# rmcar17/SpectralClusterSupertree

Hardware: AMD Instinct MI355X
Metric: top-level PCG build + Fiedler solve wall-time (s) at N taxa, 1/2/4/8 MI355X (lower is better)
Workload: dtype f64 (loop operator: fp32 image of W; fp64 renewal + confirmation)

## Files before the change

spectralclustersupertree_amd/csrc/scs_eig.hip:

```cpp

#include <algorithm>
#include <chrono>
#include <cmath>

#include "scs_internal.h"
#include "scs_policy.h"
#include "scs_symm.h"
#include "scs_matfree.h"
#include "scs_symm_tri.h"

#include <sched.h>
#include "scs_panel.h"

constexpr int MAXB = 16;
constexpr int MAXS = 64;
constexpr int SLD = MAXS + 1;

typedef double v4d __attribute__((ext_vector_type(4)));

__global__ void k_scale_rows(const double *__restrict__ x, int ldx, int c0, int b, int n,
                             const double *__restrict__ dinv, double *__restrict__ zt,
                             int64_t ldz) {
    const int idx = blockIdx.x * blockDim.x + threadIdx.x;
    if (idx >= n * b) return;
// ... 111 lines not shown
                                                          int nparts, int nout,
                                                          double *__restrict__ out) {
    const int lane = threadIdx.x & 63;
    const int e = blockIdx.x * 4 + (threadIdx.x >> 6);
    if (e >= nout) return;
    double s = 0.0;
    for (int p = lane; p < nparts; p += 64) s += partial[(int64_t)p * nout + e];
#pragma unroll
    for (int o = 32; o > 0; o >>= 1) s += __shfl_xor(s, o, 64);
    if (lane == 0) out[e] = s;
}

__global__ __launch_bounds__(256) void k_update(double *y, int ldy, int kc, double alpha_y,
                                                 const double *a, int lda, int ka,
                                                 const double *__restrict__ c, int ldc,
                                                 double sign, int n) {
    __shared__ double sc[3 * MAXB][MAXB];
    for (int e = threadIdx.x; e < ka * kc; e += 256) {
        const int i = e / kc, j = e - i * kc;
        sc[i][j] = c[i * ldc + j];
    }
    __syncthreads();
    const int r = blockIdx.x * 16 + (threadIdx.x >> 4);
    const int j = threadIdx.x & 15;
    double acc = 0.0, yold = 0.0;
    const bool live = r < n && j < kc;
    if (live) {
        const double *ar = a + (int64_t)r * lda;
        for (int i = 0; i < ka; ++i) acc += ar[i] * sc[i][j];
        if (alpha_y != 0.0) yold = y[(int64_t)r * ldy + j];
    }
    __syncthreads();
// ... 69 lines not shown
    x ^= x >> 30;
    x *= 0xBF58476D1CE4E5B9ull;
    x ^= x >> 27;
    x *= 0x94D049BB133111EBull;
    x ^= x >> 31;
    return (double)(x >> 11) * (2.0 / 9007199254740992.0) - 1.0;
}

__global__ void k_init_block(double *__restrict__ q, int b, int n, const double *__restrict__ x0) {
    const int idx = blockIdx.x * blockDim.x + threadIdx.x;
    if (idx >= n * b) return;
    const int i = idx / b, k = idx - i * b;
    double v = hash_uniform((unsigned long long)i, (unsigned long long)k + 1);
    if (k == 0 && x0) v = x0[i];
    q[(int64_t)i * (3 * b) + k] = v;
}

__global__ void k_fill_int(int *p, int n, int v) {
    const int i = blockIdx.x * blockDim.x + threadIdx.x;
    if (i < n) p[i] = v;
}

__global__ void k_trivial(const double *__restrict__ deg, double inv_norm, int n,
                          double *__restrict__ u) {
    const int i = blockIdx.x * blockDim.x + threadIdx.x;
    if (i < n) u[i] = sqrt(deg[i]) * inv_norm;
}

__global__ void k_extract_maps(const double *__restrict__ q, int ldq, int n,
                               const double *__restrict__ dinv, double inv_norm, int constrained,
                               double *__restrict__ out) {
    const int i = blockIdx.x * blockDim.x + threadIdx.x;
    if (i >= n) return;
    const double di = dinv[i];
    if (constrained) {
// ... 857 lines not shown
        const int i = e / b, k = e - i * b;
        double v = 0.0;
        for (int a = 0; a < b; ++a) v += dd[i][a] * gg[a][k];
        d[e] = v;
    }
}

__global__ __launch_bounds__(256) void k_small_rr(const double *__restrict__ tm, int nparts,
                                                   int nq, int b, const int *__restrict__ mask,
                                                   double *__restrict__ c, double *__restrict__ d,
                                                   double *__restrict__ theta,
                                                   int *__restrict__ mask_p, double drop_tol) {
    small_rr_body(tm, nparts, nq, b, mask, c, d, theta, mask_p, drop_tol);
}

struct orth_lds {
    jacobi_lds s;
    double cxp[16][8], gm[9][8], mm[8][8], tt[8][8], dsc[8];
    double tmp[8][3 * MAXB * 3 * MAXB / 4];
    __device__ void eig(int b) { jacobi_eig(s, b); }
};
template <int B>
struct orth_small_lds {
    jacobi_small_lds<B> s;
    double cxp[2 * B][B], gm[B + 1][B], mm[B][B], tt[B][B], dsc[B];
    double tmp[8][3 * B * B + B];
    double coef[PANEL_COEF_ROWS<B> * B];
    panel_red_t red;
    __device__ void eig(int) { jacobi_eig_waves<B>(s); }
};
// ... 86 lines not shown
template <int B>
__global__ __launch_bounds__(256) void k_panel_rr_solve(double *q, double *aq,
                                                         const double *__restrict__ u,
                                                         const double *__restrict__ tm, int nparts_in,
                                                         int solve, double *theta_g,
                                                         const int *__restrict__ maskp_in,
                                                         const int *__restrict__ mask_r,
                                                         int *maskp_out, double drop_tol, int n,
                                                         double *__restrict__ partial,
                                                         const double *__restrict__ dinv = nullptr,
                                                         double *__restrict__ zt = nullptr, int64_t ldz = 0,
                                                         int exact_from = -1) {
    __shared__ double c_s[3 * B * B], d_s[3 * B * B], th_s[B + 4];
    __shared__ int live_s[3 * B], mp_s[B];
    const int tid = threadIdx.x;
    if (solve) {
        if (tid < 3 * B) live_s[tid] = tid < B ? 1 : (tid < 2 * B ? maskp_in[tid - B] : mask_r[tid - 2 * B]);
        __syncthreads();
        small_rr_body(tm, nparts_in, 3 * B, B, live_s, c_s, d_s, th_s, mp_s, drop_tol, exact_from);
    } else {
        for (int e = tid; e < 3 * B * B; e += 256) {
            c_s[e] = (e / B == e % B) ? 1.0 : 0.0;
            d_s[e] = 0.0;
        }
        if (tid <= B) th_s[tid] = theta_g[tid];
        if (tid < B) mp_s[tid] = 0;
    }
    __syncthreads();
    if (blockIdx.x == 0) {
        if (solve && tid <= B) theta_g[tid] = th_s[tid];
        if (tid < B) maskp_out[tid] = mp_s[tid];
    }
    panel_rr_body<B>(q, aq, u, c_s, d_s, th_s, n, partial, dinv, zt, ldz);
}

template <int B, bool GRAM, bool WRITE_Z>
__global__ __launch_bounds__(256) void k_panel_tf_solve(double *q, const double *__restrict__ u,
                                                         const double *__restrict__ part_in,
                                                         int nparts_in, double drop_tol, int *mask_r,
                                                         const double *__restrict__ theta_g,
                                                         double *report, double seq, int n,
                                                         double *__restrict__ partial,
                                                         const double *__restrict__ dinv,
                                                         double *__restrict__ zt, int64_t ldz) {
    __shared__ double coef_s[PANEL_COEF_ROWS<B> * B];
    const bool lead = blockIdx.x == 0;
    small_orth_body(part_in, nparts_in, B, drop_tol, coef_s, lead ? mask_r : nullptr, theta_g,
                    lead ? report : nullptr, -1.0);
    __syncthreads();
    panel_tf_body<B, GRAM, WRITE_Z>(q, u, coef_s, n, partial, dinv, zt, ldz);
    if (lead && report) {
        __threadfence_system();
        __syncthreads();
        if (threadIdx.x == 0) ((volatile double *)report)[40] = seq;
    }
}

template <int B, int FINISH>
__global__ __launch_bounds__(256) void k_panel_gram_tf_solve(double *q, double *aq, const double *__restrict__ u,
                                                              const double *__restrict__ part_in, int nparts_in,
                                                              int *mask_r, const double *__restrict__ theta_g, int n,
                                                              const double *__restrict__ ypart, int nseg,
                                                              const double *__restrict__ dinv,
                                                              double *__restrict__ partial, int64_t chunk = 0,
                                                              const int32_t *__restrict__ splits = nullptr,
                                                              const double *__restrict__ coef1 = nullptr) {
    constexpr int NC = PANEL_COEF_ROWS<B> * B;
    __shared__ double coef_s[NC], coefa_s[NC];
    const bool lead = blockIdx.x == 0;
    small_orth_body(part_in, nparts_in, B, 0.0, coef_s, lead ? mask_r : nullptr, theta_g, nullptr, -1.0);
    __syncthreads();
    for (int e = threadIdx.x; e < NC; e += 256) {
        const int k = e / B, c = e - k * B;
        double v = coef_s[e];
        if (coef1) {
            if (k >= 2 * B && k < 3 * B) v = 0.0;
            for (int i = 0; i < B; ++i) v += coef1[k * B + i] * coef_s[(2 * B + i) * B + c];
        }
        coefa_s[e] = v;
    }
    __syncthreads();
    panel_gram_tf_body<B, FINISH>(q, aq, u, coef_s, coefa_s, n, ypart, nseg, dinv, partial, chunk, splits);
}

template <int B, int CT, int RPW, int D, typename WT = double>
__global__ __launch_bounds__(256, 2) void k_symm_tri_tf(const WT *__restrict__ w, int64_t ld, int n,
                                                        const double *__restrict__ zt, int64_t ldz,
                                                        const int2 *__restrict__ tiles,
                                                        double *__restrict__ pdir, double *__restrict__ ptr_,
                                                        int n_tf, double *q, const double *__restrict__ u,
                                                        const double *__restrict__ part_in, int nparts_in,
                                                        double drop_tol, int *mask_r,
                                                        const double *__restrict__ theta_g, double *report,
                                                        double seq, double *__restrict__ partial,
                                                        double *__restrict__ coef_out) {
    union lds_t {
        symm_tri_lds<B, CT, WT> symm;
        orth_small_lds<B> tf;
    };
    __shared__ lds_t lds;
    const int bid = blockIdx.x;
    if (bid >= n_tf) {
        symm_tri_body<B, CT, RPW, D, WT>(w, ld, n, zt, ldz, tiles[bid - n_tf], pdir, ptr_, 0, lds.symm);
        return;
    }
    const bool lead = bid == 0;
    small_orth_core(lds.tf, part_in, nparts_in, B, drop_tol, lds.tf.coef, lead ? mask_r : nullptr, theta_g,
                    lead ? report : nullptr, -1.0);
    __syncthreads();
    if (lead)
        for (int e = threadIdx.x; e < PANEL_COEF_ROWS<B> * B; e += 256) coef_out[e] = lds.tf.coef[e];
    panel_tf_body<B, true, false>(q, u, lds.tf.coef, n, partial, nullptr, nullptr, 0, bid, n_tf, &lds.tf.red);
    if (lead && report) {
        __threadfence_system();
        __syncthreads();
        if (threadIdx.x == 0) ((volatile double *)report)[40] = seq;
    }
}

__global__ void k_unit_coeffs(double *__restrict__ c, double *__restrict__ d, int b) {
    const int e = blockIdx.x * blockDim.x + threadIdx.x;
    if (e >= 3 * b * b) return;
    c[e] = (e / b == e % b) ? 1.0 : 0.0;
    d[e] = 0.0;
}

__global__ void k_dense_s(const double *__restrict__ w, int64_t ld, int n,
// ... 521 lines not shown
        k_gram_mfma<TA, TB><<<nparts, 64, 0, s>>>(a, lda, ka, bm, ldb, kb, n, part.d());
            GM(1, 1) GM(1, 2) GM(1, 3) GM(2, 1) GM(2, 2) GM(2, 3) GM(3, 1) GM(3, 2) GM(3, 3)
#undef GM
        } else {
            nparts = std::min(gram_blocks, std::max(1, (n + GRAM_CH - 1) / GRAM_CH));
            k_gram<<<nparts, 256, 0, s>>>(a, lda, ka, bm, ldb, kb, n, part.d());
        }
        k_reduce_partials<<<(nout + 3) / 4, 256, 0, s>>>(part.d(), nparts, nout, out);
        SCS_HIP_CHECK(hipGetLastError());
        return SCS_OK;
    }

    int update(double *y, int ldy, int kc, double alpha, const double *a, int lda, int ka,
               const double *c, int ldc, double sign) {
        k_update<<<(n + 15) / 16, 256, 0, s>>>(y, ldy, kc, alpha, a, lda, ka, c, ldc, sign, n);
        SCS_HIP_CHECK(hipGetLastError());
        return SCS_OK;
    }

    static int panel_cap() {
        static const int cap = PANEL_BLOCKS_MAX;
        return cap;
    }
    int panel_blocks16() const { return std::max(1, std::min(panel_cap(), ((n + 15) / 16 + 3) / 4)); }
    int panel_blocks4() const { return std::max(1, std::min(panel_cap(), ((n + 3) / 4 + 3) / 4)); }

    template <int B>
    int fused_front(const double *uvec, const double *c, const double *d, const double *theta,
                    double *coef, int *mask_r, double drop_tol, double *report, double seq) {
        const int nb = panel_blocks16();
// ... 356 lines not shown
        for (int pass = 0; pass < 2; ++pass) {
            SCS_TRY(sv.gram(Y, q3, b, Y, q3, b, G, sv.use_mfma));
            k_small_svqb<<<1, 256, 0, s>>>(G, b, pass == 0 ? drop_tol : 0.0, T, mask_out);
            SCS_TRY(sv.update(Y, q3, b, 0.0, Y, q3, b, T, b, 1.0));
            if (AY) SCS_TRY(sv.update(AY, q3, b, 0.0, AY, q3, b, T, b, 1.0));
        }
        return SCS_OK;
    };

    k_init_block<<<(n * b + 255) / 256, 256, 0, s>>>(Q, b, n, x_init ? x0d.d() : nullptr);
    SCS_TRY(project_u(X, 2));
    SCS_TRY(svqb(X, nullptr, MASK));
    SCS_TRY(sv.apply(Q, 0, AQ, 0));
    SCS_TRY(sv.gram(X, q3, b, AX, q3, b, G, sv.use_mfma));
    {
        k_fill_int<<<1, 64, 0, s>>>(MASK, 48, 1);
        k_small_rr<<<1, 256, 0, s>>>(G, 0, b, b, MASK, T, D, TH, MASK + b, drop_tol);
        SCS_TRY(sv.update(X, q3, b, 0.0, X, q3, b, T, b, 1.0));
        SCS_TRY(sv.update(AX, q3, b, 0.0, AX, q3, b, T, b, 1.0));
        k_fill_int<<<1, 64, 0, s>>>(MASK + b, b, 0);
    }

    const int res_blocks = (n + 255) / 256;
    dbuf res_part;
    SCS_TRY(res_part.alloc((size_t)res_blocks * b * 8));
    std::vector<double> h_rn(b), h_th(b + 1);
    int iter = 0;
    bool converged = false;
    double final_res[2] = {0.0, 0.0};

    const bool fused = (b == 4 || b == 8) &&
                       !(scs_dbg("SCS_LEGACY_LOOP") && atoi(scs_dbg("SCS_LEGACY_LOOP")));
    if (fused) {
        if (!ctx->h_report) {
            SCS_HIP_CHECK(hipHostMalloc((void **)&ctx->h_report, 64 * sizeof(double),
// ... 87 lines not shown
        }
        const int action = policy.step(worst);
        const bool stop = action == scs_loop_policy::STOP;
        if (action == scs_loop_policy::RENEW) {
            sv.use32 = false;
            SCS_TRY(sv.apply(Q, 0, AQ, 0));
            SCS_TRY(sv.apply(Q, b, AQ, b));
            sv.use32 = policy.image_in_use();
            ++st->lowp_renewals;
        }
        if (stop) {
            sv.use32 = false;
            if (policy.begin_confirmation()) {
                SCS_TRY(sv.apply(Q, 0, AQ, 0));
                SCS_TRY(sv.gram(X, q3, b, AX, q3, b, G, sv.use_mfma));
                k_fill_int<<<1, 64, 0, s>>>(MASK, 48, 1);
                k_small_rr<<<1, 256, 0, s>>>(G, 0, b, b, MASK, T, D, TH, MASK + b, drop_tol);
                SCS_TRY(sv.update(X, q3, b, 0.0, X, q3, b, T, b, 1.0));
                SCS_TRY(sv.update(AX, q3, b, 0.0, AX, q3, b, T, b, 1.0));
                k_fill_int<<<1, 64, 0, s>>>(MASK + b, b, 0);
                k_residual<<<res_blocks, 256, 0, s>>>(Q, AQ, b, TH, n, res_part.d());
                k_reduce_partials<<<(b + 3) / 4, 256, 0, s>>>(res_part.d(), res_blocks, b, RN);
                SCS_HIP_CHECK(hipMemcpyAsync(h_rn.data(), RN, (size_t)b * 8, hipMemcpyDeviceToHost, s));
                SCS_HIP_CHECK(hipMemcpyAsync(h_th.data(), TH, (size_t)(b + 1) * 8,
                                             hipMemcpyDeviceToHost, s));
                SCS_HIP_CHECK(hipStreamSynchronize(s));
                double w2 = 0.0;
                for (int j = 0; j < want; ++j) w2 = std::max(w2, std::sqrt(h_rn[j]));
                for (int j = 0; j < want; ++j) final_res[constrained ? 1 : j] = std::sqrt(h_rn[j]);
                bool conv = false;
                if (policy.confirm(w2, &conv)) {
                    converged = conv;
                    break;
                }
                if (fused) k_unit_coeffs<<<(3 * b * b + 255) / 256, 256, 0, s>>>(T, D, b);
// ... 1287 lines not shown
```

spectralclustersupertree_amd/csrc/scs_panel.h:

```cpp
#pragma once
#include <hip/hip_runtime.h>

#include <cstdint>

typedef double panel_v4d __attribute__((ext_vector_type(4)));

constexpr int PANEL_BLOCKS_MAX = 128;

template <int B>
struct panel_out {
    static constexpr int XP = 2 * B * B;
    static constexpr int RU = (B + 1) * B;
    static constexpr int TOTAL = XP + RU;
};

template <int B>
constexpr int PANEL_COEF_ROWS = 3 * B + 4;

typedef double panel_red_t[4][2][4][64];

template <int B>
__device__ __forceinline__ void panel_store_partials(panel_v4d g1, panel_v4d g2,
                                                     double *__restrict__ partial, int bid = -1,
                                                     panel_red_t *red_ext = nullptr) {
// ... 11 lines not shown
    if (wave == 0) {
        double *out = partial + (int64_t)bid * panel_out<B>::TOTAL;
#pragma unroll
        for (int r = 0; r < 4; ++r) {
            const int i = kk + 4 * r;
            const double s1 = ((red[0][0][r][lane] + red[1][0][r][lane]) + red[2][0][r][lane]) +
                              red[3][0][r][lane];
            const double s2 = ((red[0][1][r][lane] + red[1][1][r][lane]) + red[2][1][r][lane]) +
                              red[3][1][r][lane];
            if (i < 2 * B && cc < B) out[i * B + cc] = s1;
            if (i <= B && cc < B) out[panel_out<B>::XP + i * B + cc] = s2;
        }
    }
}

template <int B>
__device__ __forceinline__ void panel_rr_body(double *q, double *aq, const double *__restrict__ u,
                                              const double *c, const double *d, const double *theta,
                                              int n, double *__restrict__ partial,
                                              const double *__restrict__ dinv = nullptr,
                                              double *__restrict__ zt = nullptr, int64_t ldz = 0) {
    static_assert(B == 4 || B == 8, "fused panel kernels take block widths 4 and 8");
    constexpr int LD = 3 * B;
    const int lane = threadIdx.x & 63, wave = threadIdx.x >> 6;
    const int kk = lane >> 4, cc = lane & 15;
    const int n_groups = (n + 15) / 16;
    panel_v4d g1 = {0.0, 0.0, 0.0, 0.0}, g2 = {0.0, 0.0, 0.0, 0.0};
    const double th = cc < B ? theta[cc] : 0.0;
    double coef[LD / 4];
#pragma unroll
    for (int k = 0; k < LD / 4; ++k) {
        const int row = 4 * k + kk;
        coef[k] = cc < B ? c[row * B + cc] : (cc < 2 * B ? d[row * B + cc - B] : 0.0);
    }
    for (int grp = blockIdx.x * 4 + wave; grp < n_groups; grp += gridDim.x * 4) {
        const int base = grp * 16;
        const int ra = base + cc;
        panel_v4d dq = {0.0, 0.0, 0.0, 0.0}, da = {0.0, 0.0, 0.0, 0.0};
        double aq_op[LD / 4], q_op[LD / 4];
#pragma unroll
        for (int k = 0; k < LD / 4; ++k) {
            q_op[k] = ra < n ? q[(int64_t)ra * LD + 4 * k + kk] : 0.0;
            aq_op[k] = ra < n ? aq[(int64_t)ra * LD + 4 * k + kk] : 0.0;
        }
        double u_in[4];
#pragma unroll
        for (int r = 0; r < 4; ++r) {
            const int row = base + kk + 4 * r;
            u_in[r] = (cc == B && u && row < n) ? u[row] : 0.0;
        }
#pragma unroll
        for (int k = 0; k < LD / 4; ++k) {
            dq = __builtin_amdgcn_mfma_f64_16x16x4f64(q_op[k], coef[k], dq, 0, 0, 0);
            da = __builtin_amdgcn_mfma_f64_16x16x4f64(aq_op[k], coef[k], da, 0, 0, 0);
        }
#pragma unroll
        for (int r = 0; r < 4; ++r) {
            const int row = base + kk + 4 * r;
            const bool live = row < n;
            const double res = cc < B ? da[r] - dq[r] * th : 0.0;
            double ru = res;
            if (cc == B) ru = u_in[r];
            if (live && cc < 2 * B) {
                q[(int64_t)row * LD + cc] = dq[r];
                aq[(int64_t)row * LD + cc] = da[r];
            }
            if (live && cc < B) {
                q[(int64_t)row * LD + 2 * B + cc] = res;
                if (zt) zt[(int64_t)cc * ldz + row] = dinv[row] * res;
            }
            g1 = __builtin_amdgcn_mfma_f64_16x16x4f64(dq[r], res, g1, 0, 0, 0);
            g2 = __builtin_amdgcn_mfma_f64_16x16x4f64(ru, res, g2, 0, 0, 0);
        }
    }
    panel_store_partials<B>(g1, g2, partial);
}

template <int B>
__global__ __launch_bounds__(256) void k_panel_rr(double *q, double *aq,
                                                   const double *__restrict__ u,
                                                   const double *__restrict__ c,
                                                   const double *__restrict__ d,
                                                   const double *__restrict__ theta, int n,
                                                   double *__restrict__ partial) {
    panel_rr_body<B>(q, aq, u, c, d, theta, n, partial);
}

template <int B, bool GRAM, bool WRITE_Z>
__device__ __forceinline__ void panel_tf_body(double *q, const double *__restrict__ u,
                                              const double *coefm, int n,
                                              double *__restrict__ partial,
                                              const double *__restrict__ dinv,
                                              double *__restrict__ zt, int64_t ldz, int bid = -1,
                                              int nblk = -1, panel_red_t *red_ext = nullptr) {
    static_assert(B == 4 || B == 8, "fused panel kernels take block widths 4 and 8");
    constexpr int LD = 3 * B;
    constexpr int KC = PANEL_COEF_ROWS<B> / 4;
    if (bid < 0) {
        bid = blockIdx.x;
        nblk = gridDim.x;
    }
    const int lane = threadIdx.x & 63, wave = threadIdx.x >> 6;
    const int kk = lane >> 4, cc = lane & 15;
    const int n_groups = (n + 15) / 16;
    panel_v4d g1 = {0.0, 0.0, 0.0, 0.0}, g2 = {0.0, 0.0, 0.0, 0.0};
    double coef[KC];
#pragma unroll
    for (int k = 0; k < KC; ++k) coef[k] = cc < B ? coefm[(4 * k + kk) * B + cc] : 0.0;
    for (int grp = bid * 4 + wave; grp < n_groups; grp += nblk * 4) {
        const int base = grp * 16;
        const int ra = base + cc;
        double a_op[KC];
#pragma unroll
        for (int k = 0; k < KC - 1; ++k) a_op[k] = ra < n ? q[(int64_t)ra * LD + 4 * k + kk] : 0.0;
        a_op[KC - 1] = (kk == 0 && u && ra < n) ? u[ra] : 0.0;
        double xp_in[4], u_in[4];
        if (GRAM) {
#pragma unroll
            for (int r = 0; r < 4; ++r) {
                const int row = base + kk + 4 * r;
                xp_in[r] = (row < n && cc < 2 * B) ? q[(int64_t)row * LD + cc] : 0.0;
                u_in[r] = (cc == B && u && row < n) ? u[row] : 0.0;
            }
        }
        panel_v4d dr = {0.0, 0.0, 0.0, 0.0};
#pragma unroll
        for (int k = 0; k < KC; ++k)
            dr = __builtin_amdgcn_mfma_f64_16x16x4f64(a_op[k], coef[k], dr, 0, 0, 0);
#pragma unroll
        for (int r = 0; r < 4; ++r) {
            const int row = base + kk + 4 * r;
            const bool live = row < n;
            const double res = dr[r];
            if (live && cc < B) {
                q[(int64_t)row * LD + 2 * B + cc] = res;
                if (WRITE_Z) zt[(int64_t)cc * ldz + row] = dinv[row] * res;
            }
            if (GRAM) {
                const double xp = xp_in[r];
                double ru = res;
                if (cc == B) ru = u_in[r];
                g1 = __builtin_amdgcn_mfma_f64_16x16x4f64(xp, res, g1, 0, 0, 0);
                g2 = __builtin_amdgcn_mfma_f64_16x16x4f64(ru, res, g2, 0, 0, 0);
            }
        }
    }
    if (GRAM) panel_store_partials<B>(g1, g2, partial, bid, red_ext);
}

template <int B, bool GRAM, bool WRITE_Z>
__global__ __launch_bounds__(256) void k_panel_tf(double *q, const double *__restrict__ u,
                                                   const double *__restrict__ coefm, int n,
                                                   double *__restrict__ partial,
                                                   const double *__restrict__ dinv,
                                                   double *__restrict__ zt, int64_t ldz) {
    panel_tf_body<B, GRAM, WRITE_Z>(q, u, coefm, n, partial, dinv, zt, ldz);
}

template <int B, int FINISH>
__global__ __launch_bounds__(256) void k_gram_qaq(const double *__restrict__ q, double *aq, int n,
                                                   const double *__restrict__ ypart, int nseg,
                                                   const double *__restrict__ dinv,
// ... 79 lines not shown
#pragma unroll
        for (int i = 0; i < NT; ++i)
#pragma unroll
            for (int j = 0; j < NT; ++j)
#pragma unroll
                for (int r = 0; r < 4; ++r) {
                    const int t = i * NT + j;
                    const double s = ((red[0][t][r][lane] + red[1][t][r][lane]) + red[2][t][r][lane]) +
                                     red[3][t][r][lane];
                    const int orow = i * 16 + kk + 4 * r, ocol = j * 16 + cc;
                    if (orow < LD && ocol < LD) out[orow * LD + ocol] = s;
                }
    }
}

template <int B, int FINISH>
__device__ __forceinline__ void panel_gram_tf_body(double *q, double *aq, const double *__restrict__ u,
                                                   const double *coefm, const double *coefam, int n,
                                                   const double *__restrict__ ypart, int nseg,
                                                   const double *__restrict__ dinv,
                                                   double *__restrict__ partial, int64_t chunk,
                                                   const int32_t *__restrict__ splits) {
    static_assert(B == 4 || B == 8, "fused panel kernels take block widths 4 and 8");
    constexpr int LD = 3 * B;
    constexpr int KC = PANEL_COEF_ROWS<B> / 4;
    constexpr int NT = (LD + 15) / 16;
    constexpr int RT = (2 * B) / 16;
    constexpr int RC0 = 2 * B - 16 * RT;
    __shared__ double red[4][NT * NT][4][64];
    const int lane = threadIdx.x & 63, wave = threadIdx.x >> 6;
    const int kk = lane >> 4, cc = lane & 15;
    const int n_groups = (n + 15) / 16;
    panel_v4d acc[NT][NT];
#pragma unroll
    for (int i = 0; i < NT; ++i)
#pragma unroll
        for (int j = 0; j < NT; ++j) acc[i][j] = (panel_v4d){0.0, 0.0, 0.0, 0.0};
    double coef[KC], coefa[KC];
#pragma unroll
    for (int k = 0; k < KC; ++k) {
        const bool rc = cc >= RC0 && cc < RC0 + B;
        coef[k] = rc ? coefm[(4 * k + kk) * B + (cc - RC0)] : 0.0;
        coefa[k] = rc ? coefam[(4 * k + kk) * B + (cc - RC0)] : 0.0;
    }
    for (int grp = blockIdx.x * 4 + wave; grp < n_groups; grp += gridDim.x * 4) {
        const int base = grp * 16;
        const int ra = base + cc;
        double q_op[KC], a_op[KC];
#pragma unroll
        for (int k = 0; k < KC - 1; ++k) {
            const int col = 4 * k + kk;
            q_op[k] = ra < n ? q[(int64_t)ra * LD + col] : 0.0;
            double v = 0.0;
            if (ra < n) {
                if (col < 2 * B || FINISH == 0) {
                    v = aq[(int64_t)ra * LD + col];
                } else if (FINISH == 1) {
                    const int64_t idx = (int64_t)ra * B + (col - 2 * B);
                    double part[4];
#pragma unroll
                    for (int g = 0; g < 4; ++g) part[g] = g < nseg ? ypart[(int64_t)g * n * B + idx] : 0.0;
                    v = dinv[ra] * (((part[0] + part[1]) + part[2]) + part[3]);
                } else if (FINISH == 2) {
                    int r = 0;
                    while (r + 1 < nseg && ra >= splits[r + 1]) ++r;
                    v = ypart[(int64_t)r * chunk + (int64_t)(ra - splits[r]) * B + (col - 2 * B)];
                } else {
                    const int64_t idx = (int64_t)ra * B + (col - 2 * B);
                    double sum = 0.0;
                    for (int g = 0; g < nseg; ++g) sum += ypart[(int64_t)g * n * B + idx];
                    v = dinv[ra] * sum;
                }
            }
            a_op[k] = v;
        }
        {
            const double uu = (kk == 0 && u && ra < n) ? u[ra] : 0.0;
            q_op[KC - 1] = uu;
            a_op[KC - 1] = uu;
        }
        double xq[NT][4], xa[NT][4];
#pragma unroll
        for (int t = 0; t < NT; ++t)
#pragma unroll
            for (int r = 0; r < 4; ++r) {
                const int row = base + kk + 4 * r, col = t * 16 + cc;
                const bool live = row < n && col < 2 * B;
                xq[t][r] = live ? q[(int64_t)row * LD + col] : 0.0;
                xa[t][r] = live ? aq[(int64_t)row * LD + col] : 0.0;
            }
        panel_v4d dr = {0.0, 0.0, 0.0, 0.0}, da = {0.0, 0.0, 0.0, 0.0};
#pragma unroll
        for (int k = 0; k < KC; ++k) {
            dr = __builtin_amdgcn_mfma_f64_16x16x4f64(q_op[k], coef[k], dr, 0, 0, 0);
            da = __builtin_amdgcn_mfma_f64_16x16x4f64(a_op[k], coefa[k], da, 0, 0, 0);
        }
#pragma unroll
        for (int r = 0; r < 4; ++r) {
            const int row = base + kk + 4 * r;
            const bool rcol = cc >= RC0 && cc < RC0 + B;
            if (row < n && rcol) {
                q[(int64_t)row * LD + 2 * B + (cc - RC0)] = dr[r];
                aq[(int64_t)row * LD + 2 * B + (cc - RC0)] = da[r];
            }
            double fq[NT], fa[NT];
#pragma unroll
            for (int t = 0; t < NT; ++t) {
                fq[t] = xq[t][r];
                fa[t] = xa[t][r];
            }
            if (rcol) {
                fq[RT] = row < n ? dr[r] : 0.0;
                fa[RT] = row < n ? da[r] : 0.0;
            }
#pragma unroll
            for (int i = 0; i < NT; ++i)
#pragma unroll
                for (int j = 0; j < NT; ++j)
                    acc[i][j] = __builtin_amdgcn_mfma_f64_16x16x4f64(fq[i], fa[j], acc[i][j], 0, 0, 0);
        }
    }
#pragma unroll
    for (int i = 0; i < NT; ++i)
#pragma unroll
        for (int j = 0; j < NT; ++j)
#pragma unroll
            for (int r = 0; r < 4; ++r) red[wave][i * NT + j][r][lane] = acc[i][j][r];
    __syncthreads();
    if (wave == 0) {
        double *out = partial + (int64_t)blockIdx.x * LD * LD;
#pragma unroll
        for (int i = 0; i < NT; ++i)
#pragma unroll
            for (int j = 0; j < NT; ++j)
#pragma unroll
// ... 10 lines not shown
```

Measured before the change: 0.01418.

## Prefetch panel operands before the small Rayleigh-Ritz solve and fuse start-up kernels

The fused panel kernels now issue global loads for their first two row groups into registers before running the single-block small eigen/orthogonalisation solve, so memory latency overlaps that serial phase. The load and compute halves of the panel bodies are split into separate helpers to allow this. Separately, the start-up and confirmation Rayleigh-Ritz steps merge the mask fills and small solve into one kernel, and the two basis rotations into a single two-slice launch, cutting launch count. The cost is extra register pressure from holding the prefetched operands, which may reduce occupancy.

```diff
diff --git a/spectralclustersupertree_amd/csrc/scs_eig.hip b/spectralclustersupertree_amd/csrc/scs_eig.hip
--- a/spectralclustersupertree_amd/csrc/scs_eig.hip
+++ b/spectralclustersupertree_amd/csrc/scs_eig.hip
@@ -149,8 +149,13 @@
 __global__ __launch_bounds__(256) void k_update(double *y, int ldy, int kc, double alpha_y,
                                                  const double *a, int lda, int ka,
                                                  const double *__restrict__ c, int ldc,
-                                                 double sign, int n) {
+                                                 double sign, int n, double *y2 = nullptr,
+                                                 const double *a2 = nullptr) {
     __shared__ double sc[3 * MAXB][MAXB];
+    if (blockIdx.y) {
+        y = y2;
+        a = a2;
+    }
     for (int e = threadIdx.x; e < ka * kc; e += 256) {
         const int i = e / kc, j = e - i * kc;
         sc[i][j] = c[i * ldc + j];
@@ -250,11 +255,6 @@
     double v = hash_uniform((unsigned long long)i, (unsigned long long)k + 1);
     if (k == 0 && x0) v = x0[i];
     q[(int64_t)i * (3 * b) + k] = v;
-}
-
-__global__ void k_fill_int(int *p, int n, int v) {
-    const int i = blockIdx.x * blockDim.x + threadIdx.x;
-    if (i < n) p[i] = v;
 }
 
 __global__ void k_trivial(const double *__restrict__ deg, double inv_norm, int n,
@@ -1142,6 +1142,16 @@
     small_rr_body(tm, nparts, nq, b, mask, c, d, theta, mask_p, drop_tol);
 }
 
+__global__ __launch_bounds__(256) void k_small_rr_start(const double *__restrict__ tm, int b, int *mask,
+                                                         double *__restrict__ c, double *__restrict__ d,
+                                                         double *__restrict__ theta, double drop_tol) {
+    if (threadIdx.x < 48) mask[threadIdx.x] = 1;
+    __syncthreads();
+    small_rr_body(tm, 0, b, b, mask, c, d, theta, mask + b, drop_tol);
+    __syncthreads();
+    if ((int)threadIdx.x < b) mask[b + threadIdx.x] = 0;
+}
+
 struct orth_lds {
     jacobi_lds s;
     double cxp[16][8], gm[9][8], mm[8][8], tt[8][8], dsc[8];
@@ -1258,6 +1268,8 @@
     __shared__ double c_s[3 * B * B], d_s[3 * B * B], th_s[B + 4];
     __shared__ int live_s[3 * B], mp_s[B];
     const int tid = threadIdx.x;
+    panel_rr_ops<B> pre[PANEL_PRE];
+    panel_rr_prefetch<B>(pre, q, aq, u, dinv, zt != nullptr, n);
     if (solve) {
         if (tid < 3 * B) live_s[tid] = tid < B ? 1 : (tid < 2 * B ? maskp_in[tid - B] : mask_r[tid - 2 * B]);
         __syncthreads();
@@ -1275,7 +1287,7 @@
         if (solve && tid <= B) theta_g[tid] = th_s[tid];
         if (tid < B) maskp_out[tid] = mp_s[tid];
     }
-    panel_rr_body<B>(q, aq, u, c_s, d_s, th_s, n, partial, dinv, zt, ldz);
+    panel_rr_run<B>(pre, q, aq, u, c_s, d_s, th_s, n, partial, dinv, zt, ldz);
 }
 
 template <int B, bool GRAM, bool WRITE_Z>
@@ -1289,10 +1301,12 @@
                                                          double *__restrict__ zt, int64_t ldz) {
     __shared__ double coef_s[PANEL_COEF_ROWS<B> * B];
     const bool lead = blockIdx.x == 0;
+    panel_tf_ops<B> pre[PANEL_PRE];
+    panel_tf_prefetch<B, GRAM, WRITE_Z>(pre, q, u, dinv, n);
     small_orth_body(part_in, nparts_in, B, drop_tol, coef_s, lead ? mask_r : nullptr, theta_g,
                     lead ? report : nullptr, -1.0);
     __syncthreads();
-    panel_tf_body<B, GRAM, WRITE_Z>(q, u, coef_s, n, partial, dinv, zt, ldz);
+    panel_tf_run<B, GRAM, WRITE_Z>(pre, q, u, coef_s, n, partial, dinv, zt, ldz);
     if (lead && report) {
         __threadfence_system();
         __syncthreads();
@@ -1312,6 +1326,8 @@
     constexpr int NC = PANEL_COEF_ROWS<B> * B;
     __shared__ double coef_s[NC], coefa_s[NC];
     const bool lead = blockIdx.x == 0;
+    panel_gram_tf_ops<B> pre[PANEL_PRE];
+    panel_gram_tf_prefetch<B, FINISH>(pre, q, aq, u, n, ypart, nseg, dinv, chunk, splits);
     small_orth_body(part_in, nparts_in, B, 0.0, coef_s, lead ? mask_r : nullptr, theta_g, nullptr, -1.0);
     __syncthreads();
     for (int e = threadIdx.x; e < NC; e += 256) {
@@ -1324,7 +1340,7 @@
         coefa_s[e] = v;
     }
     __syncthreads();
-    panel_gram_tf_body<B, FINISH>(q, aq, u, coef_s, coefa_s, n, ypart, nseg, dinv, partial, chunk, splits);
+    panel_gram_tf_body<B, FINISH>(pre, q, aq, u, coef_s, coefa_s, n, ypart, nseg, dinv, partial, chunk, splits);
 }
 
 template <int B, int CT, int RPW, int D, typename WT = double>
@@ -1349,12 +1365,16 @@
         return;
     }
     const bool lead = bid == 0;
+    constexpr bool AHEAD = B == 4;
+    panel_tf_ops<B> pre[PANEL_PRE];
+    if (AHEAD) panel_tf_prefetch<B, true, false>(pre, q, u, nullptr, n, bid, n_tf);
     small_orth_core(lds.tf, part_in, nparts_in, B, drop_tol, lds.tf.coef, lead ? mask_r : nullptr, theta_g,
                     lead ? report : nullptr, -1.0);
     __syncthreads();
+    if (!AHEAD) panel_tf_prefetch<B, true, false>(pre, q, u, nullptr, n, bid, n_tf);
     if (lead)
         for (int e = threadIdx.x; e < PANEL_COEF_ROWS<B> * B; e += 256) coef_out[e] = lds.tf.coef[e];
-    panel_tf_body<B, true, false>(q, u, lds.tf.coef, n, partial, nullptr, nullptr, 0, bid, n_tf, &lds.tf.red);
+    panel_tf_run<B, true, false>(pre, q, u, lds.tf.coef, n, partial, nullptr, nullptr, 0, bid, n_tf, &lds.tf.red);
     if (lead && report) {
         __threadfence_system();
         __syncthreads();
@@ -1906,6 +1926,12 @@
     int update(double *y, int ldy, int kc, double alpha, const double *a, int lda, int ka,
                const double *c, int ldc, double sign) {
         k_update<<<(n + 15) / 16, 256, 0, s>>>(y, ldy, kc, alpha, a, lda, ka, c, ldc, sign, n);
+        SCS_HIP_CHECK(hipGetLastError());
+        return SCS_OK;
+    }
+
+    int rotate2(double *y, double *y2, int ld, int kc, const double *c, int ldc) {
+        k_update<<<dim3((n + 15) / 16, 2), 256, 0, s>>>(y, ld, kc, 0.0, y, ld, kc, c, ldc, 1.0, n, y2, y2);
         SCS_HIP_CHECK(hipGetLastError());
         return SCS_OK;
     }
@@ -2292,11 +2318,8 @@
     SCS_TRY(sv.apply(Q, 0, AQ, 0));
     SCS_TRY(sv.gram(X, q3, b, AX, q3, b, G, sv.use_mfma));
     {
-        k_fill_int<<<1, 64, 0, s>>>(MASK, 48, 1);
-        k_small_rr<<<1, 256, 0, s>>>(G, 0, b, b, MASK, T, D, TH, MASK + b, drop_tol);
-        SCS_TRY(sv.update(X, q3, b, 0.0, X, q3, b, T, b, 1.0));
-        SCS_TRY(sv.update(AX, q3, b, 0.0, AX, q3, b, T, b, 1.0));
-        k_fill_int<<<1, 64, 0, s>>>(MASK + b, b, 0);
+        k_small_rr_start<<<1, 256, 0, s>>>(G, b, MASK, T, D, TH, drop_tol);
+        SCS_TRY(sv.rotate2(X, AX, q3, b, T, b));
     }
 
     const int res_blocks = (n + 255) / 256;
@@ -2414,11 +2437,8 @@
             if (policy.begin_confirmation()) {
                 SCS_TRY(sv.apply(Q, 0, AQ, 0));
                 SCS_TRY(sv.gram(X, q3, b, AX, q3, b, G, sv.use_mfma));
-                k_fill_int<<<1, 64, 0, s>>>(MASK, 48, 1);
-                k_small_rr<<<1, 256, 0, s>>>(G, 0, b, b, MASK, T, D, TH, MASK + b, drop_tol);
-                SCS_TRY(sv.update(X, q3, b, 0.0, X, q3, b, T, b, 1.0));
-                SCS_TRY(sv.update(AX, q3, b, 0.0, AX, q3, b, T, b, 1.0));
-                k_fill_int<<<1, 64, 0, s>>>(MASK + b, b, 0);
+                k_small_rr_start<<<1, 256, 0, s>>>(G, b, MASK, T, D, TH, drop_tol);
+                SCS_TRY(sv.rotate2(X, AX, q3, b, T, b));
                 k_residual<<<res_blocks, 256, 0, s>>>(Q, AQ, b, TH, n, res_part.d());
                 k_reduce_partials<<<(b + 3) / 4, 256, 0, s>>>(res_part.d(), res_blocks, b, RN);
                 SCS_HIP_CHECK(hipMemcpyAsync(h_rn.data(), RN, (size_t)b * 8, hipMemcpyDeviceToHost, s));
diff --git a/spectralclustersupertree_amd/csrc/scs_panel.h b/spectralclustersupertree_amd/csrc/scs_panel.h
--- a/spectralclustersupertree_amd/csrc/scs_panel.h
+++ b/spectralclustersupertree_amd/csrc/scs_panel.h
@@ -49,66 +49,124 @@
     }
 }
 
+constexpr int PANEL_PRE = 2;
+
+__device__ __forceinline__ int panel_group(int bid, int nblk, int i) {
+    return bid * 4 + (int)(threadIdx.x >> 6) + i * nblk * 4;
+}
+
+template <int B>
+struct panel_rr_ops {
+    double q_op[3 * B / 4], aq_op[3 * B / 4], u_in[4], dv[4];
+};
+
+template <int B>
+__device__ __forceinline__ void panel_rr_load(panel_rr_ops<B> &o, const double *q, const double *aq,
+                                              const double *__restrict__ u,
+                                              const double *__restrict__ dinv, bool with_z, int n, int grp) {
+    constexpr int LD = 3 * B;
+    const int lane = threadIdx.x & 63;
+    const int kk = lane >> 4, cc = lane & 15;
+    const int base = grp * 16;
+    const int ra = base + cc;
+#pragma unroll
+    for (int k = 0; k < LD / 4; ++k) {
+        o.q_op[k] = ra < n ? q[(int64_t)ra * LD + 4 * k + kk] : 0.0;
+        o.aq_op[k] = ra < n ? aq[(int64_t)ra * LD + 4 * k + kk] : 0.0;
+    }
+#pragma unroll
+    for (int r = 0; r < 4; ++r) {
+        const int row = base + kk + 4 * r;
+        o.u_in[r] = (cc == B && u && row < n) ? u[row] : 0.0;
+        o.dv[r] = (with_z && cc < B && row < n) ? dinv[row] : 0.0;
+    }
+}
+
+template <int B>
+__device__ __forceinline__ void panel_rr_compute(const panel_rr_ops<B> &o, double *q, double *aq,
+                                                 const double (&coef)[3 * B / 4], double th, int n, int grp,
+                                                 double *__restrict__ zt, int64_t ldz, panel_v4d &g1,
+                                                 panel_v4d &g2) {
+    constexpr int LD = 3 * B;
+    const int lane = threadIdx.x & 63;
+    const int kk = lane >> 4, cc = lane & 15;
+    const int base = grp * 16;
+    panel_v4d dq = {0.0, 0.0, 0.0, 0.0}, da = {0.0, 0.0, 0.0, 0.0};
+#pragma unroll
+    for (int k = 0; k < LD / 4; ++k) {
+        dq = __builtin_amdgcn_mfma_f64_16x16x4f64(o.q_op[k], coef[k], dq, 0, 0, 0);
+        da = __builtin_amdgcn_mfma_f64_16x16x4f64(o.aq_op[k], coef[k], da, 0, 0, 0);
+    }
+#pragma unroll
+    for (int r = 0; r < 4; ++r) {
+        const int row = base + kk + 4 * r;
+        const bool live = row < n;
+        const double res = cc < B ? da[r] - dq[r] * th : 0.0;
+        double ru = res;
+        if (cc == B) ru = o.u_in[r];
+        if (live && cc < 2 * B) {
+            q[(int64_t)row * LD + cc] = dq[r];
+            aq[(int64_t)row * LD + cc] = da[r];
+        }
+        if (live && cc < B) {
+            q[(int64_t)row * LD + 2 * B + cc] = res;
+            if (zt) zt[(int64_t)cc * ldz + row] = o.dv[r] * res;
+        }
+        g1 = __builtin_amdgcn_mfma_f64_16x16x4f64(dq[r], res, g1, 0, 0, 0);
+        g2 = __builtin_amdgcn_mfma_f64_16x16x4f64(ru, res, g2, 0, 0, 0);
+    }
+}
+
+template <int B>
+__device__ __forceinline__ void panel_rr_prefetch(panel_rr_ops<B> (&pre)[PANEL_PRE], const double *q,
+                                                  const double *aq, const double *__restrict__ u,
+                                                  const double *__restrict__ dinv, bool with_z, int n) {
+#pragma unroll
+    for (int i = 0; i < PANEL_PRE; ++i)
+        panel_rr_load<B>(pre[i], q, aq, u, dinv, with_z, n, panel_group(blockIdx.x, gridDim.x, i));
+}
+
+template <int B>
+__device__ __forceinline__ void panel_rr_run(panel_rr_ops<B> (&pre)[PANEL_PRE], double *q, double *aq,
+                                             const double *__restrict__ u, const double *c, const double *d,
+                                             const double *theta, int n, double *__restrict__ partial,
+                                             const double *__restrict__ dinv, double *__restrict__ zt,
+                                             int64_t ldz) {
+    static_assert(B == 4 || B == 8, "fused panel kernels take block widths 4 and 8");
+    constexpr int LD = 3 * B;
+    const int lane = threadIdx.x & 63;
+    const int kk = lane >> 4, cc = lane & 15;
+    const int n_groups = (n + 15) / 16;
+    panel_v4d g1 = {0.0, 0.0, 0.0, 0.0}, g2 = {0.0, 0.0, 0.0, 0.0};
+    const double th = cc < B ? theta[cc] : 0.0;
+    double coef[LD / 4];
+#pragma unroll
+    for (int k = 0; k < LD / 4; ++k) {
+        const int row = 4 * k + kk;
+        coef[k] = cc < B ? c[row * B + cc] : (cc < 2 * B ? d[row * B + cc - B] : 0.0);
+    }
+#pragma unroll
+    for (int i = 0; i < PANEL_PRE; ++i) {
+        const int grp = panel_group(blockIdx.x, gridDim.x, i);
+        if (grp < n_groups) panel_rr_compute<B>(pre[i], q, aq, coef, th, n, grp, zt, ldz, g1, g2);
+    }
+    for (int grp = panel_group(blockIdx.x, gridDim.x, PANEL_PRE); grp < n_groups; grp += gridDim.x * 4) {
+        panel_rr_ops<B> o;
+        panel_rr_load<B>(o, q, aq, u, dinv, zt != nullptr, n, grp);
+        panel_rr_compute<B>(o, q, aq, coef, th, n, grp, zt, ldz, g1, g2);
+    }
+    panel_store_partials<B>(g1, g2, partial);
+}
+
 template <int B>
 __device__ __forceinline__ void panel_rr_body(double *q, double *aq, const double *__restrict__ u,
                                               const double *c, const double *d, const double *theta,
                                               int n, double *__restrict__ partial,
                                               const double *__restrict__ dinv = nullptr,
                                               double *__restrict__ zt = nullptr, int64_t ldz = 0) {
-    static_assert(B == 4 || B == 8, "fused panel kernels take block widths 4 and 8");
-    constexpr int LD = 3 * B;
-    const int lane = threadIdx.x & 63, wave = threadIdx.x >> 6;
-    const int kk = lane >> 4, cc = lane & 15;
-    const int n_groups = (n + 15) / 16;
-    panel_v4d g1 = {0.0, 0.0, 0.0, 0.0}, g2 = {0.0, 0.0, 0.0, 0.0};
-    const double th = cc < B ? theta[cc] : 0.0;
-    double coef[LD / 4];
-#pragma unroll
-    for (int k = 0; k < LD / 4; ++k) {
-        const int row = 4 * k + kk;
-        coef[k] = cc < B ? c[row * B + cc] : (cc < 2 * B ? d[row * B + cc - B] : 0.0);
-    }
-    for (int grp = blockIdx.x * 4 + wave; grp < n_groups; grp += gridDim.x * 4) {
-        const int base = grp * 16;
-        const int ra = base + cc;
-        panel_v4d dq = {0.0, 0.0, 0.0, 0.0}, da = {0.0, 0.0, 0.0, 0.0};
-        double aq_op[LD / 4], q_op[LD / 4];
-#pragma unroll
-        for (int k = 0; k < LD / 4; ++k) {
-            q_op[k] = ra < n ? q[(int64_t)ra * LD + 4 * k + kk] : 0.0;
-            aq_op[k] = ra < n ? aq[(int64_t)ra * LD + 4 * k + kk] : 0.0;
-        }
-        double u_in[4];
-#pragma unroll
-        for (int r = 0; r < 4; ++r) {
-            const int row = base + kk + 4 * r;
-            u_in[r] = (cc == B && u && row < n) ? u[row] : 0.0;
-        }
-#pragma unroll
-        for (int k = 0; k < LD / 4; ++k) {
-            dq = __builtin_amdgcn_mfma_f64_16x16x4f64(q_op[k], coef[k], dq, 0, 0, 0);
-            da = __builtin_amdgcn_mfma_f64_16x16x4f64(aq_op[k], coef[k], da, 0, 0, 0);
-        }
-#pragma unroll
-        for (int r = 0; r < 4; ++r) {
-            const int row = base + kk + 4 * r;
-            const bool live = row < n;
-            const double res = cc < B ? da[r] - dq[r] * th : 0.0;
-            double ru = res;
-            if (cc == B) ru = u_in[r];
-            if (live && cc < 2 * B) {
-                q[(int64_t)row * LD + cc] = dq[r];
-                aq[(int64_t)row * LD + cc] = da[r];
-            }
-            if (live && cc < B) {
-                q[(int64_t)row * LD + 2 * B + cc] = res;
-                if (zt) zt[(int64_t)cc * ldz + row] = dinv[row] * res;
-            }
-            g1 = __builtin_amdgcn_mfma_f64_16x16x4f64(dq[r], res, g1, 0, 0, 0);
-            g2 = __builtin_amdgcn_mfma_f64_16x16x4f64(ru, res, g2, 0, 0, 0);
-        }
-    }
-    panel_store_partials<B>(g1, g2, partial);
+    panel_rr_ops<B> pre[PANEL_PRE];
+    panel_rr_prefetch<B>(pre, q, aq, u, dinv, zt != nullptr, n);
+    panel_rr_run<B>(pre, q, aq, u, c, d, theta, n, partial, dinv, zt, ldz);
 }
 
 template <int B>
@@ -121,6 +179,111 @@
     panel_rr_body<B>(q, aq, u, c, d, theta, n, partial);
 }
 
+template <int B>
+struct panel_tf_ops {
+    double a_op[PANEL_COEF_ROWS<B> / 4], xp_in[4], u_in[4], dv[4];
+};
+
+template <int B, bool GRAM, bool WRITE_Z>
+__device__ __forceinline__ void panel_tf_load(panel_tf_ops<B> &o, const double *q,
+                                              const double *__restrict__ u,
+                                              const double *__restrict__ dinv, int n, int grp) {
+    constexpr int LD = 3 * B;
+    constexpr int KC = PANEL_COEF_ROWS<B> / 4;
+    const int lane = threadIdx.x & 63;
+    const int kk = lane >> 4, cc = lane & 15;
+    const int base = grp * 16;
+    const int ra = base + cc;
+#pragma unroll
+    for (int k = 0; k < KC - 1; ++k) o.a_op[k] = ra < n ? q[(int64_t)ra * LD + 4 * k + kk] : 0.0;
+    o.a_op[KC - 1] = (kk == 0 && u && ra < n) ? u[ra] : 0.0;
+#pragma unroll
+    for (int r = 0; r < 4; ++r) {
+        const int row = base + kk + 4 * r;
+        o.xp_in[r] = (GRAM && row < n && cc < 2 * B) ? q[(int64_t)row * LD + cc] : 0.0;
+        o.u_in[r] = (GRAM && cc == B && u && row < n) ? u[row] : 0.0;
+        o.dv[r] = (WRITE_Z && row < n && cc < B) ? dinv[row] : 0.0;
+    }
+}
+
+template <int B, bool GRAM, bool WRITE_Z>
+__device__ __forceinline__ void panel_tf_compute(const panel_tf_ops<B> &o, double *q,
+                                                 const double (&coef)[PANEL_COEF_ROWS<B> / 4], int n, int grp,
+                                                 double *__restrict__ zt, int64_t ldz, panel_v4d &g1,
+                                                 panel_v4d &g2) {
+    constexpr int LD = 3 * B;
+    constexpr int KC = PANEL_COEF_ROWS<B> / 4;
+    const int lane = threadIdx.x & 63;
+    const int kk = lane >> 4, cc = lane & 15;
+    const int base = grp * 16;
+    panel_v4d dr = {0.0, 0.0, 0.0, 0.0};
+#pragma unroll
+    for (int k = 0; k < KC; ++k) dr = __builtin_amdgcn_mfma_f64_16x16x4f64(o.a_op[k], coef[k], dr, 0, 0, 0);
+#pragma unroll
+    for (int r = 0; r < 4; ++r) {
+        const int row = base + kk + 4 * r;
+        const bool live = row < n;
+        const double res = dr[r];
+        if (live && cc < B) {
+            q[(int64_t)row * LD + 2 * B + cc] = res;
+            if (WRITE_Z) zt[(int64_t)cc * ldz + row] = o.dv[r] * res;
+        }
+        if (GRAM) {
+            const double xp = o.xp_in[r];
+            double ru = res;
+            if (cc == B) ru = o.u_in[r];
+            g1 = __builtin_amdgcn_mfma_f64_16x16x4f64(xp, res, g1, 0, 0, 0);
+            g2 = __builtin_amdgcn_mfma_f64_16x16x4f64(ru, res, g2, 0, 0, 0);
+        }
+    }
+}
+
+template <int B, bool GRAM, bool WRITE_Z>
+__device__ __forceinline__ void panel_tf_prefetch(panel_tf_ops<B> (&pre)[PANEL_PRE], const double *q,
+                                                  const double *__restrict__ u,
+                                                  const double *__restrict__ dinv, int n, int bid = -1,
+                                                  int nblk = -1) {
+    if (bid < 0) {
+        bid = blockIdx.x;
+        nblk = gridDim.x;
+    }
+#pragma unroll
+    for (int i = 0; i < PANEL_PRE; ++i)
+        panel_tf_load<B, GRAM, WRITE_Z>(pre[i], q, u, dinv, n, panel_group(bid, nblk, i));
+}
+
+template <int B, bool GRAM, bool WRITE_Z>
+__device__ __forceinline__ void panel_tf_run(panel_tf_ops<B> (&pre)[PANEL_PRE], double *q,
+                                             const double *__restrict__ u, const double *coefm, int n,
+                                             double *__restrict__ partial, const double *__restrict__ dinv,
+                                             double *__restrict__ zt, int64_t ldz, int bid = -1, int nblk = -1,
+                                             panel_red_t *red_ext = nullptr) {
+    static_assert(B == 4 || B == 8, "fused panel kernels take block widths 4 and 8");
+    constexpr int KC = PANEL_COEF_ROWS<B> / 4;
+    if (bid < 0) {
+        bid = blockIdx.x;
+        nblk = gridDim.x;
+    }
+    const int lane = threadIdx.x & 63;
+    const int kk = lane >> 4, cc = lane & 15;
+    const int n_groups = (n + 15) / 16;
+    panel_v4d g1 = {0.0, 0.0, 0.0, 0.0}, g2 = {0.0, 0.0, 0.0, 0.0};
+    double coef[KC];
+#pragma unroll
+    for (int k = 0; k < KC; ++k) coef[k] = cc < B ? coefm[(4 * k + kk) * B + cc] : 0.0;
+#pragma unroll
+    for (int i = 0; i < PANEL_PRE; ++i) {
+        const int grp = panel_group(bid, nblk, i);
+        if (grp < n_groups) panel_tf_compute<B, GRAM, WRITE_Z>(pre[i], q, coef, n, grp, zt, ldz, g1, g2);
+    }
+    for (int grp = panel_group(bid, nblk, PANEL_PRE); grp < n_groups; grp += nblk * 4) {
+        panel_tf_ops<B> o;
+        panel_tf_load<B, GRAM, WRITE_Z>(o, q, u, dinv, n, grp);
+        panel_tf_compute<B, GRAM, WRITE_Z>(o, q, coef, n, grp, zt, ldz, g1, g2);
+    }
+    if (GRAM) panel_store_partials<B>(g1, g2, partial, bid, red_ext);
+}
+
 template <int B, bool GRAM, bool WRITE_Z>
 __device__ __forceinline__ void panel_tf_body(double *q, const double *__restrict__ u,
                                               const double *coefm, int n,
@@ -128,59 +291,9 @@
                                               const double *__restrict__ dinv,
                                               double *__restrict__ zt, int64_t ldz, int bid = -1,
                                               int nblk = -1, panel_red_t *red_ext = nullptr) {
-    static_assert(B == 4 || B == 8, "fused panel kernels take block widths 4 and 8");
-    constexpr int LD = 3 * B;
-    constexpr int KC = PANEL_COEF_ROWS<B> / 4;
-    if (bid < 0) {
-        bid = blockIdx.x;
-        nblk = gridDim.x;
-    }
-    const int lane = threadIdx.x & 63, wave = threadIdx.x >> 6;
-    const int kk = lane >> 4, cc = lane & 15;
-    const int n_groups = (n + 15) / 16;
-    panel_v4d g1 = {0.0, 0.0, 0.0, 0.0}, g2 = {0.0, 0.0, 0.0, 0.0};
-    double coef[KC];
-#pragma unroll
-    for (int k = 0; k < KC; ++k) coef[k] = cc < B ? coefm[(4 * k + kk) * B + cc] : 0.0;
-    for (int grp = bid * 4 + wave; grp < n_groups; grp += nblk * 4) {
-        const int base = grp * 16;
-        const int ra = base + cc;
-        double a_op[KC];
-#pragma unroll
-        for (int k = 0; k < KC - 1; ++k) a_op[k] = ra < n ? q[(int64_t)ra * LD + 4 * k + kk] : 0.0;
-        a_op[KC - 1] = (kk == 0 && u && ra < n) ? u[ra] : 0.0;
-        double xp_in[4], u_in[4];
-        if (GRAM) {
-#pragma unroll
-            for (int r = 0; r < 4; ++r) {
-                const int row = base + kk + 4 * r;
-                xp_in[r] = (row < n && cc < 2 * B) ? q[(int64_t)row * LD + cc] : 0.0;
-                u_in[r] = (cc == B && u && row < n) ? u[row] : 0.0;
-            }
-        }
-        panel_v4d dr = {0.0, 0.0, 0.0, 0.0};
-#pragma unroll
-        for (int k = 0; k < KC; ++k)
-            dr = __builtin_amdgcn_mfma_f64_16x16x4f64(a_op[k], coef[k], dr, 0, 0, 0);
-#pragma unroll
-        for (int r = 0; r < 4; ++r) {
-            const int row = base + kk + 4 * r;
-            const bool live = row < n;
-            const double res = dr[r];
-            if (live && cc < B) {
-                q[(int64_t)row * LD + 2 * B + cc] = res;
-                if (WRITE_Z) zt[(int64_t)cc * ldz + row] = dinv[row] * res;
-            }
-            if (GRAM) {
-                const double xp = xp_in[r];
-                double ru = res;
-                if (cc == B) ru = u_in[r];
-                g1 = __builtin_amdgcn_mfma_f64_16x16x4f64(xp, res, g1, 0, 0, 0);
-                g2 = __builtin_amdgcn_mfma_f64_16x16x4f64(ru, res, g2, 0, 0, 0);
-            }
-        }
-    }
-    if (GRAM) panel_store_partials<B>(g1, g2, partial, bid, red_ext);
+    panel_tf_ops<B> pre[PANEL_PRE];
+    panel_tf_prefetch<B, GRAM, WRITE_Z>(pre, q, u, dinv, n, bid, nblk);
+    panel_tf_run<B, GRAM, WRITE_Z>(pre, q, u, coefm, n, partial, dinv, zt, ldz, bid, nblk, red_ext);
 }
 
 template <int B, bool GRAM, bool WRITE_Z>
@@ -290,8 +403,140 @@
     }
 }
 
+template <int B>
+struct panel_gram_tf_ops {
+    static constexpr int KC = PANEL_COEF_ROWS<B> / 4;
+    static constexpr int NT = (3 * B + 15) / 16;
+    double q_op[KC], a_op[KC];
+    double part[B / 4][4], dv;
+    double xq[NT][4], xa[NT][4];
+};
+
 template <int B, int FINISH>
-__device__ __forceinline__ void panel_gram_tf_body(double *q, double *aq, const double *__restrict__ u,
+__device__ __forceinline__ void panel_gram_tf_load(panel_gram_tf_ops<B> &o, const double *q, const double *aq,
+                                                   const double *__restrict__ u, int n,
+                                                   const double *__restrict__ ypart, int nseg,
+                                                   const double *__restrict__ dinv, int64_t chunk,
+                                                   const int32_t *__restrict__ splits, int grp) {
+    constexpr int LD = 3 * B;
+    constexpr int KC = PANEL_COEF_ROWS<B> / 4;
+    constexpr int NT = (LD + 15) / 16;
+    constexpr int KR = 2 * B / 4;
+    const int lane = threadIdx.x & 63;
+    const int kk = lane >> 4, cc = lane & 15;
+    const int base = grp * 16;
+    const int ra = base + cc;
+    o.dv = (FINISH == 1 && ra < n) ? dinv[ra] : 0.0;
+#pragma unroll
+    for (int k = 0; k < KC - 1; ++k) {
+        const int col = 4 * k + kk;
+        o.q_op[k] = ra < n ? q[(int64_t)ra * LD + col] : 0.0;
+        double v = 0.0;
+        if (k < KR || FINISH == 0) {
+            if (ra < n) v = aq[(int64_t)ra * LD + col];
+        } else if (FINISH == 1) {
+            const int64_t idx = (int64_t)ra * B + (col - 2 * B);
+#pragma unroll
+            for (int g = 0; g < 4; ++g)
+                o.part[k - KR][g] = (ra < n && g < nseg) ? ypart[(int64_t)g * n * B + idx] : 0.0;
+        } else if (ra < n) {
+            if (FINISH == 2) {
+                int r = 0;
+                while (r + 1 < nseg && ra >= splits[r + 1]) ++r;
+                v = ypart[(int64_t)r * chunk + (int64_t)(ra - splits[r]) * B + (col - 2 * B)];
+            } else {
+                const int64_t idx = (int64_t)ra * B + (col - 2 * B);
+                double sum = 0.0;
+                for (int g = 0; g < nseg; ++g) sum += ypart[(int64_t)g * n * B + idx];
+                v = dinv[ra] * sum;
+            }
+        }
+        o.a_op[k] = v;
+    }
+    {
+        const double uu = (kk == 0 && u && ra < n) ? u[ra] : 0.0;
+        o.q_op[KC - 1] = uu;
+        o.a_op[KC - 1] = uu;
+    }
+#pragma unroll
+    for (int t = 0; t < NT; ++t)
+#pragma unroll
+        for (int r = 0; r < 4; ++r) {
+            const int row = base + kk + 4 * r, col = t * 16 + cc;
+            const bool live = row < n && col < 2 * B;
+            o.xq[t][r] = live ? q[(int64_t)row * LD + col] : 0.0;
+            o.xa[t][r] = live ? aq[(int64_t)row * LD + col] : 0.0;
+        }
+}
+
+template <int B, int FINISH>
+__device__ __forceinline__ void panel_gram_tf_prefetch(panel_gram_tf_ops<B> (&pre)[PANEL_PRE], const double *q,
+                                                       const double *aq, const double *__restrict__ u, int n,
+                                                       const double *__restrict__ ypart, int nseg,
+                                                       const double *__restrict__ dinv, int64_t chunk,
+                                                       const int32_t *__restrict__ splits) {
+#pragma unroll
+    for (int i = 0; i < PANEL_PRE; ++i)
+        panel_gram_tf_load<B, FINISH>(pre[i], q, aq, u, n, ypart, nseg, dinv, chunk, splits,
+                                      panel_group(blockIdx.x, gridDim.x, i));
+}
+
+template <int B, int FINISH>
+__device__ __forceinline__ void panel_gram_tf_compute(panel_gram_tf_ops<B> &o, double *q, double *aq,
+                                                      const double (&coef)[PANEL_COEF_ROWS<B> / 4],
+                                                      const double (&coefa)[PANEL_COEF_ROWS<B> / 4], int n, int grp,
+                                                      panel_v4d (&acc)[(3 * B + 15) / 16][(3 * B + 15) / 16]) {
+    constexpr int LD = 3 * B;
+    constexpr int KC = PANEL_COEF_ROWS<B> / 4;
+    constexpr int NT = (LD + 15) / 16;
+    constexpr int RT = (2 * B) / 16;
+    constexpr int RC0 = 2 * B - 16 * RT;
+    constexpr int KR = 2 * B / 4;
+    const int lane = threadIdx.x & 63;
+    const int kk = lane >> 4, cc = lane & 15;
+    const int base = grp * 16;
+    if (FINISH == 1) {
+#pragma unroll
+        for (int k = KR; k < KC - 1; ++k) {
+            const double *part = o.part[k - KR];
+            o.a_op[k] = o.dv * (((part[0] + part[1]) + part[2]) + part[3]);
+        }
+    }
+    panel_v4d dr = {0.0, 0.0, 0.0, 0.0}, da = {0.0, 0.0, 0.0, 0.0};
+#pragma unroll
+    for (int k = 0; k < KC; ++k) {
+        dr = __builtin_amdgcn_mfma_f64_16x16x4f64(o.q_op[k], coef[k], dr, 0, 0, 0);
+        da = __builtin_amdgcn_mfma_f64_16x16x4f64(o.a_op[k], coefa[k], da, 0, 0, 0);
+    }
+#pragma unroll
+    for (int r = 0; r < 4; ++r) {
+        const int row = base + kk + 4 * r;
+        const bool rcol = cc >= RC0 && cc < RC0 + B;
+        if (row < n && rcol) {
+            q[(int64_t)row * LD + 2 * B + (cc - RC0)] = dr[r];
+            aq[(int64_t)row * LD + 2 * B + (cc - RC0)] = da[r];
+        }
+        double fq[NT], fa[NT];
+#pragma unroll
+        for (int t = 0; t < NT; ++t) {
+            fq[t] = o.xq[t][r];
+            fa[t] = o.xa[t][r];
+        }
+        if (rcol) {
+            fq[RT] = row < n ? dr[r] : 0.0;
+            fa[RT] = row < n ? da[r] : 0.0;
+        }
+#pragma unroll
+        for (int i = 0; i < NT; ++i)
+#pragma unroll
+            for (int j = 0; j < NT; ++j)
+                acc[i][j] = __builtin_amdgcn_mfma_f64_16x16x4f64(fq[i], fa[j], acc[i][j], 0, 0, 0);
+    }
+}
+
+template <int B, int FINISH>
+__device__ __forceinline__ void panel_gram_tf_body(panel_gram_tf_ops<B> (&pre)[PANEL_PRE], double *q,
+                                                   double *aq, const double *__restrict__ u,
                                                    const double *coefm, const double *coefam, int n,
                                                    const double *__restrict__ ypart, int nseg,
                                                    const double *__restrict__ dinv,
@@ -319,82 +564,15 @@
         coef[k] = rc ? coefm[(4 * k + kk) * B + (cc - RC0)] : 0.0;
         coefa[k] = rc ? coefam[(4 * k + kk) * B + (cc - RC0)] : 0.0;
     }
-    for (int grp = blockIdx.x * 4 + wave; grp < n_groups; grp += gridDim.x * 4) {
-        const int base = grp * 16;
-        const int ra = base + cc;
-        double q_op[KC], a_op[KC];
-#pragma unroll
-        for (int k = 0; k < KC - 1; ++k) {
-            const int col = 4 * k + kk;
-            q_op[k] = ra < n ? q[(int64_t)ra * LD + col] : 0.0;
-            double v = 0.0;
-            if (ra < n) {
-                if (col < 2 * B || FINISH == 0) {
-                    v = aq[(int64_t)ra * LD + col];
-                } else if (FINISH == 1) {
-                    const int64_t idx = (int64_t)ra * B + (col - 2 * B);
-                    double part[4];
-#pragma unroll
-                    for (int g = 0; g < 4; ++g) part[g] = g < nseg ? ypart[(int64_t)g * n * B + idx] : 0.0;
-                    v = dinv[ra] * (((part[0] + part[1]) + part[2]) + part[3]);
-                } else if (FINISH == 2) {
-                    int r = 0;
-                    while (r + 1 < nseg && ra >= splits[r + 1]) ++r;
-                    v = ypart[(int64_t)r * chunk + (int64_t)(ra - splits[r]) * B + (col - 2 * B)];
-                } else {
-                    const int64_t idx = (int64_t)ra * B + (col - 2 * B);
-                    double sum = 0.0;
-                    for (int g = 0; g < nseg; ++g) sum += ypart[(int64_t)g * n * B + idx];
-                    v = dinv[ra] * sum;
-                }
-            }
-            a_op[k] = v;
-        }
-        {
-            const double uu = (kk == 0 && u && ra < n) ? u[ra] : 0.0;
-            q_op[KC - 1] = uu;
-            a_op[KC - 1] = uu;
-        }
-        double xq[NT][4], xa[NT][4];
-#pragma unroll
-        for (int t = 0; t < NT; ++t)
-#pragma unroll
-            for (int r = 0; r < 4; ++r) {
-                const int row = base + kk + 4 * r, col = t * 16 + cc;
-                const bool live = row < n && col < 2 * B;
-                xq[t][r] = live ? q[(int64_t)row * LD + col] : 0.0;
-                xa[t][r] = live ? aq[(int64_t)row * LD + col] : 0.0;
-            }
-        panel_v4d dr = {0.0, 0.0, 0.0, 0.0}, da = {0.0, 0.0, 0.0, 0.0};
-#pragma unroll
-        for (int k = 0; k < KC; ++k) {
-            dr = __builtin_amdgcn_mfma_f64_16x16x4f64(q_op[k], coef[k], dr, 0, 0, 0);
-            da = __builtin_amdgcn_mfma_f64_16x16x4f64(a_op[k], coefa[k], da, 0, 0, 0);
-        }
-#pragma unroll
-        for (int r = 0; r < 4; ++r) {
-            const int row = base + kk + 4 * r;
-            const bool rcol = cc >= RC0 && cc < RC0 + B;
-            if (row < n && rcol) {
-                q[(int64_t)row * LD + 2 * B + (cc - RC0)] = dr[r];
-                aq[(int64_t)row * LD + 2 * B + (cc - RC0)] = da[r];
-            }
-            double fq[NT], fa[NT];
-#pragma unroll
-            for (int t = 0; t < NT; ++t) {
-                fq[t] = xq[t][r];
-                fa[t] = xa[t][r];
-            }
-            if (rcol) {
-                fq[RT] = row < n ? dr[r] : 0.0;
-                fa[RT] = row < n ? da[r] : 0.0;
-            }
-#pragma unroll
-            for (int i = 0; i < NT; ++i)
-#pragma unroll
-                for (int j = 0; j < NT; ++j)
-                    acc[i][j] = __builtin_amdgcn_mfma_f64_16x16x4f64(fq[i], fa[j], acc[i][j], 0, 0, 0);
-        }
+#pragma unroll
+    for (int i = 0; i < PANEL_PRE; ++i) {
+        const int grp = panel_group(blockIdx.x, gridDim.x, i);
+        if (grp < n_groups) panel_gram_tf_compute<B, FINISH>(pre[i], q, aq, coef, coefa, n, grp, acc);
+    }
+    for (int grp = panel_group(blockIdx.x, gridDim.x, PANEL_PRE); grp < n_groups; grp += gridDim.x * 4) {
+        panel_gram_tf_ops<B> o;
+        panel_gram_tf_load<B, FINISH>(o, q, aq, u, n, ypart, nseg, dinv, chunk, splits, grp);
+        panel_gram_tf_compute<B, FINISH>(o, q, aq, coef, coefa, n, grp, acc);
     }
 #pragma unroll
     for (int i = 0; i < NT; ++i)
```

Measured after the change: 0.01397, median of 6. 1.5% less time.
